# thiagopbueno/tf-mpc

Measured on AMD Instinct MI355X. Metric: iLQR iterations/sec (batch x horizon) at n=16,m=8,T=50, higher is better.
Workload: dtype f32

## Files before the change

tf-mpc_amd/csrc/lqr_mfma16x8.hip:

```cpp
#include <hip/hip_runtime.h>

#include <cstdlib>
#include <cstring>
#include <type_traits>

#include "lqr_kernels.h"
#include "options.h"
#include "mfma_bf16x3.h"
#include "wave_ldlt8.h"
#include "wave_ldlt8_pair.h"
#include "wave_ops.h"

namespace tfmpc {

namespace {

constexpr int N = 16, M = 8, D = 24;
using f32x4 = bf3::f32x4;

__device__ __forceinline__ f32x4 mfma(float a, float b, f32x4 c)
{
    return __builtin_amdgcn_mfma_f32_16x16x4f32(a, b, c, 0, 0, 0);
}

__device__ __forceinline__ float readlane(float v, int lane)
{
    return __builtin_bit_cast(float, __builtin_amdgcn_readlane(__builtin_bit_cast(int, v), lane));
}

using namespace bf3;

constexpr int kMs = 0;
constexpr int kKs = 256;
constexpr int kVt = 512;
constexpr int kVtLd = 20;
constexpr int kSweepFloats = kVt + 16 * kVtLd;
constexpr int kZs = 0;
constexpr int kZld = 26;
#ifndef TFMPC_LQR_TC
#define TFMPC_LQR_TC 52
#endif
constexpr int kTC = TFMPC_LQR_TC;
constexpr int kRolloutFloats = kZs + (kTC + 1) * kZld + 6;
constexpr int kLdsFloats = kSweepFloats > kRolloutFloats ? kSweepFloats : kRolloutFloats;
static_assert(kLdsFloats % 4 == 0, "slices are 16-byte aligned (pair_src, the 16-byte accesses of the sweep)");
#ifndef TFMPC_LQR_RING
#define TFMPC_LQR_RING 4
#endif
constexpr int kRing = TFMPC_LQR_RING;
static_assert(kTC % kRing == 0, "a chunk must hold whole turns of the gain ring");

template <int CTRL>
__device__ __forceinline__ float dpp(float v)
{
    return __builtin_bit_cast(float, __builtin_amdgcn_update_dpp(0, __builtin_bit_cast(int, v), CTRL, 0xF, 0xF, false));
}
constexpr int kDppXor1 = 0xB1;
constexpr int kDppXor2 = 0x4E;
constexpr int kDppHalfMirror = 0x141;

#define TFMPC_GLOBAL __attribute__((address_space(1)))
#define TFMPC_LDS __attribute__((address_space(3)))
using gbytes = TFMPC_GLOBAL char *;
__device__ __forceinline__ gbytes uniform_base(const float *p)
{
    gbytes g = (gbytes)p;
    asm("" : "+s"(g));
    return g;
}
__device__ __forceinline__ unsigned here(unsigned &off)
{
    asm volatile("" : "+v"(off));
    return off;
}
template <class V>
__device__ __forceinline__ V gload(gbytes base, unsigned &off) { return *reinterpret_cast<const TFMPC_GLOBAL V *>(base + here(off)); }
template <class V>
__device__ __forceinline__ void gstore(gbytes base, unsigned &off, V v) { *reinterpret_cast<TFMPC_GLOBAL V *>(base + here(off)) = v; }
__device__ __forceinline__ int pinned(int v)
{
    asm("" : "+v"(v));
    return v;
}
typedef float f32x4_lds __attribute__((ext_vector_type(4), aligned(8)));
typedef float f32x4_any __attribute__((ext_vector_type(4), aligned(4)));

#ifdef TFMPC_LQR_EU
#define TFMPC_LQR_WAVES(EU_) TFMPC_LQR_EU
#else
#define TFMPC_LQR_WAVES(EU_) (EU_)
#endif
#define TFMPC_LQR_OCCUPANCY __attribute__((amdgpu_waves_per_eu(TFMPC_LQR_WAVES(EU), TFMPC_LQR_WAVES(EU))))
__device__ __forceinline__ void block_lds_sync()
{
    __builtin_amdgcn_fence(__ATOMIC_RELEASE, "workgroup", "local");
    __builtin_amdgcn_s_barrier();
    __builtin_amdgcn_fence(__ATOMIC_ACQUIRE, "workgroup", "local");
}
template <bool BACKWARD, bool FORWARD, bool VALUE, bool EXACT, bool BF3, bool OUT16 = false, int EU = 4, bool PAIR = false>
__global__ __launch_bounds__(PAIR ? 2 * kWave : kWave) TFMPC_LQR_OCCUPANCY void lqr_mfma16x8_kernel(LqrArgs a)
{
    static_assert(!PAIR || (BACKWARD && !VALUE && !OUT16), "the paired elimination serves the sweeps without value outputs");
    __shared__ __attribute__((aligned(16))) float lds_all[(PAIR ? 2 : 1) * kLdsFloats];
    const int wave = PAIR ? __builtin_amdgcn_readfirstlane(threadIdx.x >> 6) : 0;
    float *const lds = lds_all + wave * kLdsFloats;
    const int b_own = PAIR ? 2 * (int)blockIdx.x + wave : (int)blockIdx.x;
    const bool live = !PAIR || b_own < a.B;
    const int b = live ? b_own : a.B - 1;
    const int lane = PAIR ? (int)(threadIdx.x & (kWave - 1)) : (int)threadIdx.x;
    const int i = lane & 15, q = lane >> 4;
    const int T = a.T;
    const int n = EXACT ? N : a.n, m = EXACT ? M : a.m, d = n + m;
    auto Fxx = [&](const float *Fg, int row, int xi) { return (row < n && xi < n) ? Fg[row * d + xi] : 0.0f; };
    auto Fxu = [&](const float *Fg, int row, int ui) { return (row < n && ui < m) ? Fg[row * d + n + ui] : 0.0f; };
    auto zmap = [&](int zi) { return zi < N ? (zi < n ? zi : -1) : (zi - N < m ? n + zi - N : -1); };
    auto Czz = [&](const float *Cg, int zr, int zc) {
        const int r = zmap(zr), c_ = zmap(zc);
        return (r >= 0 && c_ >= 0) ? Cg[r * d + c_] : 0.0f;
    };
    auto cz = [&](const float *cg, int zr) { const int r = zmap(zr); return r >= 0 ? cg[r] : 0.0f; };
    const float *Fg = a.F + (size_t)b * a.sF;
    const float *fg = a.f + (size_t)b * a.sf;
    const float *Cg = a.C + (size_t)b * a.sC;
    const float *cg = a.c + (size_t)b * a.sc;
    float *Kg = a.K + (size_t)b * a.sK;
    float *kg = a.k + (size_t)b * a.sk;
    int status = 0;

    if (BACKWARD) {
        float Fb0[4], Fb1[4];
        f32x4 Cd00, Cd11;
        f32x4 Cd01t;
        f32x4 vterm;
#pragma unroll
        for (int r = 0; r < 4; ++r) {
            const int k = 4 * q + r;
            const int ku = N + k;
            if (EXACT) {
                Fb0[r] = Fg[k * D + i];
                Fb1[r] = (i < M) ? Fg[k * D + N + i] : ((i == M) ? fg[k] : 0.0f);
                Cd00[r] = Cg[k * D + i];
                Cd01t[r] = (k < M) ? Cg[(N + k) * D + i] : ((k == M) ? cg[i] : 0.0f);
                vterm[r] = (i == M) ? cg[k] : 0.0f;
                Cd11[r] = (ku < D) ? ((i < M) ? Cg[ku * D + N + i] : ((i == M) ? cg[ku] : 0.0f)) : 0.0f;
            } else {
                Fb0[r] = Fxx(Fg, k, i);
                Fb1[r] = (i < M) ? Fxu(Fg, k, i) : ((i == M && k < n) ? fg[k] : 0.0f);
                Cd00[r] = Czz(Cg, k, i);
                Cd01t[r] = (k < M) ? Czz(Cg, N + k, i) : ((k == M) ? cz(cg, i) : 0.0f);
                vterm[r] = (i == M) ? cz(cg, k) : 0.0f;
                float c11 = 0.0f;
                if (ku < D) {
                    if (i < M) c11 = (k >= m && i == k) ? 1.0f : Czz(Cg, ku, N + i);
                    else if (i == M) c11 = cz(cg, ku);
                }
                Cd11[r] = c11;
            }
        }
        ConstFrag Fc0{}, Fc1{};
        if (BF3) {
            Fc0 = const_frag(f32x4{Fb0[0], Fb0[1], Fb0[2], Fb0[3]});
            Fc1 = const_frag(f32x4{Fb1[0], Fb1[1], Fb1[2], Fb1[3]});
        }
        f32x4 Vd = Cd00, vd = vterm;
        float cst = 0.0f;
        int min_pivot_bits = 0x3f800000;
        int min_pivot_rows = 0x3f800000;
        const int pj = lane & 15, prow = (lane >> 4) & 1;
        const int pcol = pj >= 8 ? pj - 8 + 8 * prow : (pj == 0 ? N + M : N + pj);
        const int pair_src = PAIR ? 4 * pinned(((lane >> 5) * kLdsFloats + kMs + pcol * 8) / 4) : 0;
        const int pair_d0 = (lane >> 5) * kLdsFloats + kMs + N * 8;
        constexpr int kZero = kMs + 25 * 8;
        if (lane < kKs - kZero) lds[kZero + lane] = 0.0f;
        constexpr int kQx = kMs + 28 * 8;
        constexpr int kPark = kMs + 30 * 8;
        const int pair_qx = (lane >> 5) * kLdsFloats + (pj >= 8 ? kQx + pj - 8 + 8 * prow : kPark + pj + 8 * prow);
        const int t01_src = (i == M) ? kQx + 4 * q : kZero;
        const int g0_src = pinned(kKs + i * 8 + q);
        const int vt_dst = pinned(kVt + 4 * q * kVtLd + i);
        unsigned offK = 8u * lane, offk = 4u * lane;
        __syncthreads();

        auto sweep_step = [&](const int t, auto LAST) __attribute__((always_inline)) {
            f32x4 W0 = {0.f, 0.f, 0.f, 0.f}, W1 = vd;
            if (BF3) {
                const VarFrag Vf = var_frag_block(Vd);
                W0 = mm_var_const(Vf, Fc0, W0);
                W1 = mm_var_const(Vf, Fc1, W1);
            } else {
#pragma unroll
                for (int r = 0; r < 4; ++r) {
                    W0 = mfma(Vd[r], Fb0[r], W0);
                    W1 = mfma(Vd[r], Fb1[r], W1);
                }
            }
            float fw = 0.0f, fv = 0.0f;
            if (VALUE) {
                float pw = 0.0f, pv = 0.0f;
#pragma unroll
                for (int r = 0; r < 4; ++r) {
                    pw = fmaf(Fb1[r], W1[r], pw);
                    pv = fmaf(Fb1[r], vd[r], pv);
                }
                fw = wave_sum(i == M ? pw : 0.0f);
                fv = wave_sum(i == M ? pv : 0.0f);
            }
            f32x4 T00 = Cd00, T01t = Cd01t, T11 = Cd11;
            if (BF3) {
                const VarFrag W0f = var_frag_block(W0), W1f = var_frag_block(W1);
                T00 = mm_const_var(Fc0, W0f, T00);
                T01t = mm_var_const(W1f, Fc0, T01t);
                T11 = mm_const_var(Fc1, W1f, T11);
            } else {
#pragma unroll
                for (int r = 0; r < 4; ++r) {
                    T00 = mfma(Fb0[r], W0[r], T00);
                    T01t = mfma(W1[r], Fb0[r], T01t);
                    T11 = mfma(Fb1[r], W1[r], T11);
                }
            }
            if (q < 2) {
                *reinterpret_cast<f32x4 *>(&lds[kMs + i * 8 + 4 * q]) = T01t;
                if (i <= M) *reinterpret_cast<f32x4 *>(&lds[kMs + (N + i) * 8 + 4 * q]) = T11;
            } else if (q == 2) {
                lds[kQx + i] = T01t[0];
            }
            float quk = 0.0f;
            if constexpr (PAIR) {
                block_lds_sync();
                if (wave == (t & 1)) {
                    f32x2 P2[4];
                    const f32x4 lo = *reinterpret_cast<const f32x4 *>(&lds_all[pair_src]);
                    const f32x4 hi = *reinterpret_cast<const f32x4 *>(&lds_all[pair_src + 4]);
                    const float d0 = lds_all[pair_d0];
                    const f32x4 qlo = *(const volatile TFMPC_LDS f32x4 *)&lds_all[pair_src];
                    const f32x4 qhi = *(const volatile TFMPC_LDS f32x4 *)&lds_all[pair_src + 4];
                    float vnext = lds_all[pair_qx];
                    P2[0] = f32x2{lo[0], lo[1]}; P2[1] = f32x2{lo[2], lo[3]};
                    P2[2] = f32x2{hi[0], hi[1]}; P2[3] = f32x2{hi[2], hi[3]};
                    const float Qc[8] = {qlo[0], qlo[1], qlo[2], qlo[3], qhi[0], qhi[1], qhi[2], qhi[3]};
                    float Pr[8];
                    ldlt8_pair_solve_neg(P2, Pr, d0, min_pivot_rows, Qc, vnext);
                    lds_all[pair_qx] = vnext;
                    f32x4 klo, khi;
#pragma unroll
                    for (int r = 0; r < 4; ++r) { klo[r] = Pr[r]; khi[r] = Pr[4 + r]; }
                    *reinterpret_cast<f32x4 *>(&lds_all[pair_src + (kKs - kMs)]) = klo;
                    *reinterpret_cast<f32x4 *>(&lds_all[pair_src + (kKs - kMs) + 4]) = khi;
                }
                block_lds_sync();
            } else {
                lds_sync();
                f32x2 M2[4];
                float Qc[8];
                {
                    const int c = lane & 31;
                    const f32x4 lo = *reinterpret_cast<const f32x4 *>(&lds[kMs + c * 8]);
                    const f32x4 hi = *reinterpret_cast<const f32x4 *>(&lds[kMs + c * 8 + 4]);
                    M2[0] = f32x2{lo[0], lo[1]}; M2[1] = f32x2{lo[2], lo[3]};
                    M2[2] = f32x2{hi[0], hi[1]}; M2[3] = f32x2{hi[2], hi[3]};
#pragma unroll
                    for (int r = 0; r < 4; ++r) { Qc[r] = lo[r]; Qc[4 + r] = hi[r]; }
                }
                float vnext = lds[kQx + (lane & 15)];
                float qu_saved[8];
                if (VALUE) {
#pragma unroll
                    for (int p = 0; p < 8; ++p) qu_saved[p] = readlane(M2[p >> 1][p & 1], 24);
                }
                float Mr[8];
                ldlt8_solve_neg(M2, Mr, min_pivot_bits);
                float kb[8];
#pragma unroll
                for (int p = 0; p < 8; ++p) kb[p] = readlane(Mr[p], 24);
                if (VALUE) {
#pragma unroll
                    for (int p = 0; p < 8; ++p) quk = fmaf(kb[p], qu_saved[p], quk);
                }
                if constexpr (!decltype(LAST)::value) {
#pragma unroll
                    for (int p = 0; p < 8; ++p) vnext = fmaf(kb[p], Qc[p], vnext);
                    if (lane < N) lds[kQx + lane] = vnext;
                }
                if (lane < 32) {
                    f32x4 lo, hi;
#pragma unroll
                    for (int r = 0; r < 4; ++r) { lo[r] = Mr[r]; hi[r] = Mr[4 + r]; }
                    *reinterpret_cast<f32x4 *>(&lds[kKs + lane * 8]) = lo;
                    *reinterpret_cast<f32x4 *>(&lds[kKs + lane * 8 + 4]) = hi;
                }
                lds_sync();
            }
            if constexpr (!decltype(LAST)::value) {
                const f32x4 vacc = *reinterpret_cast<const f32x4 *>(&lds[t01_src]);
#pragma unroll
                for (int s2 = 0; s2 < 2; ++s2) {
                    const float ax = lds[kMs + i * 8 + 4 * s2 + q];
                    const float g0 = lds[g0_src + 4 * s2];
                    T00 = mfma(ax, g0, T00);
                }
                {
                    const float *vt = &lds[kVt];
#pragma unroll
                    for (int r = 0; r < 4; ++r) lds[vt_dst + r * kVtLd] = T00[r];
                    lds_sync();
                    const f32x4 Tt = *reinterpret_cast<const f32x4 *>(&vt[i * kVtLd + 4 * q]);
#pragma unroll
                    for (int r = 0; r < 4; ++r) Vd[r] = 0.5f * (T00[r] + Tt[r]);
                }
                vd = vacc;
            }
            if (live) {
                const int ka = lane >> 3, jc = lane & 7;
                float2 kv;
                kv.x = lds[kKs + (2 * jc) * 8 + ka];
                kv.y = lds[kKs + (2 * jc + 1) * 8 + ka];
                if (EXACT) {
                    gstore(uniform_base(Kg + (size_t)t * (M * N)), offK, f32x2{kv.x, kv.y});
                    if (lane < M) gstore(uniform_base(kg + (size_t)t * M), offk, lds[kKs + 24 * 8 + lane]);
                } else {
                    if (ka < m && 2 * jc < n) Kg[(size_t)t * m * n + ka * n + 2 * jc] = kv.x;
                    if (ka < m && 2 * jc + 1 < n) Kg[(size_t)t * m * n + ka * n + 2 * jc + 1] = kv.y;
                    if (lane < m) kg[(size_t)t * m + lane] = lds[kKs + 24 * 8 + lane];
                }
                if (OUT16 && a.K16) {
                    uint16_t *Ko = a.K16 + ((size_t)b * T + t) * (m * n);
                    if (ka < m && 2 * jc < n) Ko[ka * n + 2 * jc] = lqr_to_bf16(kv.x);
                    if (ka < m && 2 * jc + 1 < n) Ko[ka * n + 2 * jc + 1] = lqr_to_bf16(kv.y);
                }
                if (OUT16 && a.k16 && lane < m) a.k16[((size_t)b * T + t) * m + lane] = lqr_to_bf16(lds[kKs + 24 * 8 + lane]);
            }
            if (VALUE) {
                cst += 0.5f * quk + 0.5f * (fw + fv);
                if (a.V) {
                    float *Vo = a.V + ((size_t)b * T + t) * (n * n);
#pragma unroll
                    for (int r = 0; r < 4; ++r)
                        if (EXACT || (4 * q + r < n && i < n)) Vo[(4 * q + r) * n + i] = Vd[r];
                }
                if (a.v && i == M) {
                    float *vo = a.v + ((size_t)b * T + t) * n;
#pragma unroll
                    for (int r = 0; r < 4; ++r)
                        if (EXACT || 4 * q + r < n) vo[4 * q + r] = vd[r];
                }
                if (a.cst && lane == 0) a.cst[(size_t)b * T + t] = cst;
                if (OUT16 && a.V16) {
                    uint16_t *Vo = a.V16 + ((size_t)b * T + t) * (n * n);
#pragma unroll
                    for (int r = 0; r < 4; ++r)
                        if (EXACT || (4 * q + r < n && i < n)) Vo[(4 * q + r) * n + i] = lqr_to_bf16(Vd[r]);
                }
                if (OUT16 && a.v16 && i == M) {
                    uint16_t *vo = a.v16 + ((size_t)b * T + t) * n;
#pragma unroll
                    for (int r = 0; r < 4; ++r)
                        if (EXACT || 4 * q + r < n) vo[4 * q + r] = lqr_to_bf16(vd[r]);
                }
                if (OUT16 && a.cst16 && lane == 0) a.cst16[(size_t)b * T + t] = lqr_to_bf16(cst);
            }
            lds_sync();
        };
        constexpr int kPeeled = VALUE ? 0 : 1;
        for (int t = T - 1; t >= kPeeled; --t) sweep_step(t, std::false_type{});
        if (kPeeled && T > 0) sweep_step(0, std::true_type{});
        if constexpr (PAIR) {
            constexpr int kMinPv = kKs + 25 * 8;
            if ((lane & 31) == 0) lds[kMinPv + (lane >> 5)] = __builtin_bit_cast(float, min_pivot_rows);
            block_lds_sync();
            const int p0 = __builtin_bit_cast(int, lds_all[kMinPv + wave]), p1 = __builtin_bit_cast(int, lds_all[kLdsFloats + kMinPv + wave]);
            min_pivot_bits = __builtin_amdgcn_readfirstlane(p0 < p1 ? p0 : p1);
        }
        if (min_pivot_bits <= 0) status |= (min_pivot_bits == 0) ? TFMPC_ST_SINGULAR : TFMPC_ST_NOT_PD;
        if (VALUE && !(cst == cst)) status |= TFMPC_ST_NAN;
    }

    const int lane_rollout = (BACKWARD && FORWARD) ? pinned((int)__builtin_amdgcn_mbcnt_hi(~0u, __builtin_amdgcn_mbcnt_lo(~0u, 0u))) : lane;
    if (FORWARD) {
        const int lane = lane_rollout, i = lane & 15, q = lane >> 4;
        const int fi = lane >> 2, fc = lane & 3;
        const int ka = lane >> 3, jc = lane & 7;
        float Fr[6];
        if (EXACT) {
            const float2 *p = reinterpret_cast<const float2 *>(Fg + fi * D + 6 * fc);
#pragma unroll
            for (int j = 0; j < 3; ++j) { const float2 v = p[j]; Fr[2 * j] = v.x; Fr[2 * j + 1] = v.y; }
        } else {
#pragma unroll
            for (int j = 0; j < 6; ++j) {
                const int zc = 6 * fc + j;
                Fr[j] = zc < N ? Fxx(Fg, fi, zc) : Fxu(Fg, fi, zc - N);
            }
        }
        const float f_part = (fc == 0 && (EXACT || fi < n)) ? fg[fi] : 0.0f;
        float Ca0[6], Ca1[6];
        f32x4 cq0, cq1;
#pragma unroll
        for (int s2 = 0; s2 < 6; ++s2) {
            if (EXACT) {
                Ca0[s2] = Cg[i * D + 4 * s2 + q];
                Ca1[s2] = (i < M) ? Cg[(N + i) * D + 4 * s2 + q] : 0.0f;
            } else {
                Ca0[s2] = Czz(Cg, i, 4 * s2 + q);
                Ca1[s2] = (i < M) ? Czz(Cg, N + i, 4 * s2 + q) : 0.0f;
            }
        }
#pragma unroll
        for (int r = 0; r < 4; ++r) {
            cq0[r] = EXACT ? cg[4 * q + r] : cz(cg, 4 * q + r);
            cq1[r] = (q < 2) ? (EXACT ? cg[N + 4 * q + r] : cz(cg, N + 4 * q + r)) : 0.0f;
        }
        float *xs = a.states + (size_t)b * (T + 1) * n;
        float *us = a.actions + (size_t)b * T * m;
        float *cs = a.costs + (size_t)b * (T + 1);
        float *zs = &lds[kZs];
        __syncthreads();
        if (lane < N) {
            const float x = (EXACT || lane < n) ? a.x0[(size_t)b * n + lane] : 0.0f;
            zs[lane] = x;
            if (live && (EXACT || lane < n)) xs[lane] = x;
        }
        unsigned offK = 8u * lane, offk = 4u * ka;
        auto load_gain = [&](int t, float2 &Kv, float &kv) {
            if (EXACT) {
                const f32x2 K2 = gload<f32x2>(uniform_base(Kg + (size_t)t * (M * N)), offK);
                Kv = float2{K2[0], K2[1]};
                kv = gload<float>(uniform_base(kg + (size_t)t * M), offk);
            } else {
                const bool row = ka < m;
                Kv.x = (row && 2 * jc < n) ? Kg[(size_t)t * m * n + ka * n + 2 * jc] : 0.0f;
                Kv.y = (row && 2 * jc + 1 < n) ? Kg[(size_t)t * m * n + ka * n + 2 * jc + 1] : 0.0f;
                kv = row ? kg[(size_t)t * m + ka] : 0.0f;
            }
        };
        float2 KR[kRing];
        float kR[kRing];
#pragma unroll
        for (int d = 0; d < kRing; ++d) {
            KR[d] = float2{0.f, 0.f};
            kR[d] = 0.0f;
            if (T > 0) load_gain(d < T ? d : T - 1, KR[d], kR[d]);
        }
        __syncthreads();

        auto chunk_costs = [&](int rows, float *out) {
            float part = 0.0f;
            for (int nt = 0; nt * 16 < rows; ++nt) {
                const int row = (16 * nt + i < rows) ? 16 * nt + i : rows - 1;
                const float *zrow = zs + row * kZld;
                f32x4 D0 = {0.f, 0.f, 0.f, 0.f}, D1 = {0.f, 0.f, 0.f, 0.f};
#pragma unroll
                for (int s2 = 0; s2 < 6; ++s2) {
                    const float bz = zrow[4 * s2 + q];
                    D0 = mfma(Ca0[s2], bz, D0);
                    D1 = mfma(Ca1[s2], bz, D1);
                }
                part = 0.0f;
#pragma unroll
                for (int r = 0; r < 4; ++r) {
                    part = fmaf(zrow[4 * q + r], fmaf(0.5f, D0[r], cq0[r]), part);
                    if (q < 2) part = fmaf(zrow[N + 4 * q + r], fmaf(0.5f, D1[r], cq1[r]), part);
                }
                part += __shfl_xor(part, 16, kWave);
                part += __shfl_xor(part, 32, kWave);
                if (live && q == 0 && 16 * nt + i < rows) {
                    unsigned offc = 4u * lane;
                    gstore(uniform_base(out + 16 * nt), offc, part);
                }
            }
            return part;
        };

        auto rollout_step = [&](const int tt, const int t, float2 &KRd, float &kRd, auto REFILL) __attribute__((always_inline)) {
            float *zt = zs + tt * kZld;
            const float2 Kc = KRd;
            const float kc = kRd;
            const float2 xv = *reinterpret_cast<const float2 *>(&zt[2 * jc]);
            float u = fmaf(Kc.x, xv.x, Kc.y * xv.y);
            u += dpp<kDppXor1>(u);
            u += dpp<kDppXor2>(u);
            u += dpp<kDppHalfMirror>(u);
            u += kc;
            if constexpr (decltype(REFILL)::value) load_gain(t + kRing < T ? t + kRing : T - 1, KRd, kRd);
            zt[N + ka] = u;
            lds_sync();
            float xn = f_part;
            const float2 *zp = reinterpret_cast<const float2 *>(&zt[6 * fc]);
#pragma unroll
            for (int j = 0; j < 3; ++j) {
                const float2 z2 = zp[j];
                xn = fmaf(Fr[2 * j], z2.x, xn);
                xn = fmaf(Fr[2 * j + 1], z2.y, xn);
            }
            xn += dpp<kDppXor1>(xn);
            xn += dpp<kDppXor2>(xn);
            zt[kZld + fi] = xn;
            lds_sync();
        };

        const int xrow = lane >> 2, urow = lane >> 1;
        const float *xsrc = zs + (1 + xrow) * kZld + 4 * (lane & 3);
        const float *usrc = zs + urow * kZld + N + 4 * (lane & 1);
        unsigned off16 = 16u * lane;
        auto rows_left = [](int v) { asm("" : "+s"(v)); return v; };

        for (int t0 = 0; t0 == 0 || t0 < T; t0 += kTC) {
            const bool last = T - t0 <= kTC;
            const int tc = last ? T - t0 : kTC;
            int tb = 0;
            for (; tb + kRing <= tc; tb += kRing) {
#pragma unroll
                for (int d = 0; d < kRing; ++d) rollout_step(tb + d, t0 + tb + d, KR[d], kR[d], std::true_type{});
            }
#pragma unroll
            for (int d = 0; d < kRing - 1; ++d)
                if (tb + d < tc) rollout_step(tb + d, t0 + tb + d, KR[d], kR[d], std::false_type{});
            if (last) {
                if (lane < M) zs[tc * kZld + N + lane] = __builtin_bit_cast(float, pinned(0));
                lds_sync();
            }
            const float tile_costs = chunk_costs(last ? tc + 1 : tc, cs + t0);
            if (last) {
                const float fcost = readlane(tile_costs, tc & 15);
                if (!(fcost == fcost)) status |= TFMPC_ST_NAN;
            }
            if (!live) {
            } else if (EXACT) {
                const gbytes xdst = uniform_base(xs + (size_t)(t0 + 1) * N), udst = uniform_base(us + (size_t)t0 * M);
#pragma unroll
                for (int r0 = 0; r0 < kTC; r0 += kWave / 4) {
                    const int left = rows_left(tc - r0);
                    if (left <= 0) break;
                    if (xrow < left)
                        gstore<f32x4_any>(xdst + r0 * (N * 4), off16, *reinterpret_cast<const f32x4_lds *>(xsrc + r0 * kZld));
                }
#pragma unroll
                for (int r0 = 0; r0 < kTC; r0 += kWave / 2) {
                    const int left = rows_left(tc - r0);
                    if (left <= 0) break;
                    if (urow < left)
                        gstore<f32x4_any>(udst + r0 * (M * 4), off16, *reinterpret_cast<const f32x4_lds *>(usrc + r0 * kZld));
                }
            } else {
                for (int idx = lane; idx < tc * n; idx += kWave)
                    xs[(size_t)(t0 + 1) * n + idx] = zs[(1 + idx / n) * kZld + idx % n];
                for (int idx = lane; idx < tc * m; idx += kWave)
                    us[(size_t)t0 * m + idx] = zs[(idx / m) * kZld + N + idx % m];
            }
            if (!last) {
                lds_sync();
                if (lane < N) zs[lane] = zs[kTC * kZld + lane];
                lds_sync();
            }
        }
    }

    if (live && a.status && lane_rollout == 0) a.status[b] = status;
}

bool use_bf16x3()
{
    return !option_is(kOptLqrMfma, "f32");
}

int pick_eu()
{
    const int forced = option_int(kOptLqrWaves, 0);
    return forced == 4 || forced == 6 ? forced : 5;
}

template <bool BW, bool FW, bool VAL, bool O16, int EU>
int launch_eu(const LqrArgs &a, hipStream_t stream)
{
    const bool exact = a.n == N && a.m == M;
    const bool bf3 = BW && use_bf16x3();
    constexpr bool P = BW && !VAL && !O16;
    const dim3 grid(P ? (a.B + 1) / 2 : a.B), block(P ? 2 * kWave : kWave);
    if (exact && bf3) hipLaunchKernelGGL((lqr_mfma16x8_kernel<BW, FW, VAL, true, true, O16, EU, P>), grid, block, 0, stream, a);
    else if (exact) hipLaunchKernelGGL((lqr_mfma16x8_kernel<BW, FW, VAL, true, false, O16, EU, P>), grid, block, 0, stream, a);
    else if (bf3) hipLaunchKernelGGL((lqr_mfma16x8_kernel<BW, FW, VAL, false, true, O16, EU, P>), grid, block, 0, stream, a);
    else hipLaunchKernelGGL((lqr_mfma16x8_kernel<BW, FW, VAL, false, false, O16, EU, P>), grid, block, 0, stream, a);
    return hipGetLastError() == hipSuccess ? TFMPC_OK : TFMPC_ERR_LAUNCH;
}

template <bool BW, bool FW, bool VAL, bool O16 = false>
int launch(const LqrArgs &a, hipStream_t stream)
{
    if constexpr (!VAL) {
        const int eu = pick_eu();
        if constexpr (BW && !O16) {
            if (eu == 6) return launch_eu<BW, FW, VAL, O16, 6>(a, stream);
        }
        if (eu >= 5) return launch_eu<BW, FW, VAL, O16, 5>(a, stream);
    }
    return launch_eu<BW, FW, VAL, O16, 4>(a, stream);
}

}

bool lqr_mfma_supported(int n, int m) { return n >= 1 && m >= 1 && n <= N && m <= M && n + m > 6; }

int lqr_mfma_launch(const LqrArgs &a, bool backward, bool forward, hipStream_t stream)
{
    if (a.K16 || a.k16 || a.V16 || a.v16 || a.cst16) {
        if (backward && forward) return launch<true, true, true, true>(a, stream);
        if (backward) return launch<true, false, true, true>(a, stream);
    }
    const bool value = a.V || a.v || a.cst;
    if (backward && forward) return value ? launch<true, true, true>(a, stream) : launch<true, true, false>(a, stream);
    if (backward) return value ? launch<true, false, true>(a, stream) : launch<true, false, false>(a, stream);
    return launch<false, true, false>(a, stream);
}

}
```

tf-mpc_amd/csrc/wave_ldlt8_pair.h:

```cpp
#pragma once

#include <hip/hip_runtime.h>

#include "wave_ldlt8.h"

namespace tfmpc {

#define TFMPC_BC(L) " row_newbcast:" #L " row_mask:0xf bank_mask:0xf\n\t"
#define TFMPC_PIVOT(P) "v_rcp_f32_dpp %[x" #P "], -%[m" #P "]" TFMPC_BC(P) \
                       "v_min_i32_dpp %[mp], %[m" #P "], %[mp]" TFMPC_BC(P) \
                       "v_mul_f32 %[x" #P "], %[m" #P "], %[x" #P "]\n\t"
#define TFMPC_FWD(P, S) "v_fmac_f32_dpp %[m" #S "], %[x" #P "], %[m" #P "]" TFMPC_BC(S)
#define TFMPC_BWD(P, O, S) "v_fmac_f32_dpp %[x" #P "], %[" #O "], %[x" #S "]" TFMPC_BC(S)
#define TFMPC_COPY(O, P) "v_mov_b32 %[" #O "], %[x" #P "]\n\t"
#define TFMPC_VAL(A) "v_fmac_f32_dpp %[acc], %[x" #A "], %[q" #A "]" TFMPC_BC(0)

__device__ __forceinline__ void ldlt8_pair_solve_neg(const f32x2 (&M2)[4], float (&X)[8], float d0, int &min_pivot_bits, const float (&Q)[8],
                                                     float &acc)
{
    float M[8];
#pragma unroll
    for (int r = 0; r < 8; ++r) M[r] = M2[r >> 1][r & 1];
    asm("v_rcp_f32 %[x0], -%[d0]\n\t"
        "v_min_i32 %[mp], %[d0], %[mp]\n\t"
        "v_mul_f32 %[x0], %[m0], %[x0]\n\t"
        "s_nop 1\n\t"
        TFMPC_FWD(0, 1) TFMPC_FWD(0, 2) TFMPC_FWD(0, 3) TFMPC_FWD(0, 4) TFMPC_FWD(0, 5) TFMPC_FWD(0, 6) TFMPC_FWD(0, 7)
        TFMPC_PIVOT(1) "s_nop 1\n\t"
        TFMPC_FWD(1, 2) TFMPC_FWD(1, 3) TFMPC_FWD(1, 4) TFMPC_FWD(1, 5) TFMPC_FWD(1, 6) TFMPC_FWD(1, 7)
        TFMPC_PIVOT(2) "s_nop 1\n\t"
        TFMPC_FWD(2, 3) TFMPC_FWD(2, 4) TFMPC_FWD(2, 5) TFMPC_FWD(2, 6) TFMPC_FWD(2, 7)
        TFMPC_PIVOT(3) "s_nop 1\n\t"
        TFMPC_FWD(3, 4) TFMPC_FWD(3, 5) TFMPC_FWD(3, 6) TFMPC_FWD(3, 7)
        TFMPC_PIVOT(4) "s_nop 1\n\t"
        TFMPC_FWD(4, 5) TFMPC_FWD(4, 6) TFMPC_FWD(4, 7)
        TFMPC_PIVOT(5) "s_nop 1\n\t"
        TFMPC_FWD(5, 6) TFMPC_FWD(5, 7)
        "s_nop 0\n\t"
        TFMPC_PIVOT(6) "s_nop 1\n\t"
        TFMPC_FWD(6, 7)
        TFMPC_COPY(m0, 5) TFMPC_COPY(m1, 4)
        TFMPC_PIVOT(7)
        "v_fmac_f32_dpp %[x6], %[x6], %[x7]" TFMPC_BC(7)
        TFMPC_BWD(5, m0, 7) TFMPC_BWD(5, m0, 6)
        TFMPC_COPY(m0, 3)
        TFMPC_BWD(4, m1, 7) TFMPC_BWD(4, m1, 6) TFMPC_BWD(4, m1, 5)
        TFMPC_COPY(m1, 2)
        TFMPC_BWD(3, m0, 7) TFMPC_BWD(3, m0, 6) TFMPC_BWD(3, m0, 5) TFMPC_BWD(3, m0, 4)
        TFMPC_COPY(m0, 1)
        TFMPC_BWD(2, m1, 7) TFMPC_BWD(2, m1, 6) TFMPC_BWD(2, m1, 5) TFMPC_BWD(2, m1, 4) TFMPC_BWD(2, m1, 3)
        TFMPC_COPY(m1, 0)
        TFMPC_BWD(1, m0, 7) TFMPC_BWD(1, m0, 6) TFMPC_BWD(1, m0, 5) TFMPC_BWD(1, m0, 4) TFMPC_BWD(1, m0, 3) TFMPC_BWD(1, m0, 2)
        TFMPC_BWD(0, m1, 7) TFMPC_BWD(0, m1, 6) TFMPC_BWD(0, m1, 5) TFMPC_BWD(0, m1, 4) TFMPC_BWD(0, m1, 3) TFMPC_BWD(0, m1, 2) TFMPC_BWD(0, m1, 1)
        "s_nop 1\n\t"
        TFMPC_VAL(0) TFMPC_VAL(1) TFMPC_VAL(2) TFMPC_VAL(3) TFMPC_VAL(4) TFMPC_VAL(5) TFMPC_VAL(6) TFMPC_VAL(7)
        : [x0] "=&v"(X[0]), [x1] "=&v"(X[1]), [x2] "=&v"(X[2]), [x3] "=&v"(X[3]), [x4] "=&v"(X[4]), [x5] "=&v"(X[5]), [x6] "=&v"(X[6]),
          [x7] "=&v"(X[7]), [m0] "+v"(M[0]), [m1] "+v"(M[1]), [m2] "+v"(M[2]), [m3] "+v"(M[3]), [m4] "+v"(M[4]), [m5] "+v"(M[5]),
          [m6] "+v"(M[6]), [m7] "+v"(M[7]), [mp] "+v"(min_pivot_bits), [acc] "+v"(acc)
        : [d0] "v"(d0), [q0] "v"(Q[0]), [q1] "v"(Q[1]), [q2] "v"(Q[2]), [q3] "v"(Q[3]), [q4] "v"(Q[4]), [q5] "v"(Q[5]), [q6] "v"(Q[6]),
          [q7] "v"(Q[7]));
}
#undef TFMPC_VAL
#undef TFMPC_COPY
#undef TFMPC_BWD
#undef TFMPC_FWD
#undef TFMPC_PIVOT
#undef TFMPC_BC

}
```

Before: 44.54 million.

## Compute value-gradient correction from eliminated rows, overlapping with LDLT solve

The value-vector update (Qx + K^T Qu) is rewritten as a dot product between the forward-eliminated rows and the original M rows, so it no longer waits for back-substitution. In the pair path the VAL accumulations are interleaved into the pivot stalls in place of s_nop padding, and the separate Q register copies read through volatile LDS loads are removed. In the single-wave path the solve is split into eliminate and backsub helpers so the vnext store can be issued before back-substitution. This shortens the critical path per timestep but changes the floating-point evaluation order, and the new eliminate and backsub helpers replace the previous tuned solve.

```diff
diff --git a/tf-mpc_amd/csrc/lqr_mfma16x8.hip b/tf-mpc_amd/csrc/lqr_mfma16x8.hip
--- a/tf-mpc_amd/csrc/lqr_mfma16x8.hip
+++ b/tf-mpc_amd/csrc/lqr_mfma16x8.hip
@@ -233,15 +233,13 @@
                     const f32x4 lo = *reinterpret_cast<const f32x4 *>(&lds_all[pair_src]);
                     const f32x4 hi = *reinterpret_cast<const f32x4 *>(&lds_all[pair_src + 4]);
                     const float d0 = lds_all[pair_d0];
-                    const f32x4 qlo = *(const volatile TFMPC_LDS f32x4 *)&lds_all[pair_src];
-                    const f32x4 qhi = *(const volatile TFMPC_LDS f32x4 *)&lds_all[pair_src + 4];
                     float vnext = lds_all[pair_qx];
                     P2[0] = f32x2{lo[0], lo[1]}; P2[1] = f32x2{lo[2], lo[3]};
                     P2[2] = f32x2{hi[0], hi[1]}; P2[3] = f32x2{hi[2], hi[3]};
-                    const float Qc[8] = {qlo[0], qlo[1], qlo[2], qlo[3], qhi[0], qhi[1], qhi[2], qhi[3]};
                     float Pr[8];
-                    ldlt8_pair_solve_neg(P2, Pr, d0, min_pivot_rows, Qc, vnext);
-                    lds_all[pair_qx] = vnext;
+                    float corr = 0.0f;
+                    ldlt8_pair_solve_neg(P2, Pr, d0, min_pivot_rows, corr);
+                    lds_all[pair_qx] = vnext + corr;
                     f32x4 klo, khi;
 #pragma unroll
                     for (int r = 0; r < 4; ++r) { klo[r] = Pr[r]; khi[r] = Pr[4 + r]; }
@@ -252,15 +250,12 @@
             } else {
                 lds_sync();
                 f32x2 M2[4];
-                float Qc[8];
                 {
                     const int c = lane & 31;
                     const f32x4 lo = *reinterpret_cast<const f32x4 *>(&lds[kMs + c * 8]);
                     const f32x4 hi = *reinterpret_cast<const f32x4 *>(&lds[kMs + c * 8 + 4]);
                     M2[0] = f32x2{lo[0], lo[1]}; M2[1] = f32x2{lo[2], lo[3]};
                     M2[2] = f32x2{hi[0], hi[1]}; M2[3] = f32x2{hi[2], hi[3]};
-#pragma unroll
-                    for (int r = 0; r < 4; ++r) { Qc[r] = lo[r]; Qc[4 + r] = hi[r]; }
                 }
                 float vnext = lds[kQx + (lane & 15)];
                 float qu_saved[8];
@@ -268,19 +263,24 @@
 #pragma unroll
                     for (int p = 0; p < 8; ++p) qu_saved[p] = readlane(M2[p >> 1][p & 1], 24);
                 }
+                f32x2 N2[4];
+                float nl[8][8];
+                ldlt8_eliminate_neg(M2, N2, nl, min_pivot_bits);
+                if constexpr (!decltype(LAST)::value) {
+                    float corr = 0.0f;
+#pragma unroll
+                    for (int p = 0; p < 8; ++p) corr = fmaf(readlane(N2[p >> 1][p & 1], 24), M2[p >> 1][p & 1], corr);
+                    vnext += corr;
+                    if (lane < N) lds[kQx + lane] = vnext;
+                }
                 float Mr[8];
-                ldlt8_solve_neg(M2, Mr, min_pivot_bits);
+                ldlt8_backsub_neg(N2, nl, Mr);
                 float kb[8];
 #pragma unroll
                 for (int p = 0; p < 8; ++p) kb[p] = readlane(Mr[p], 24);
                 if (VALUE) {
 #pragma unroll
                     for (int p = 0; p < 8; ++p) quk = fmaf(kb[p], qu_saved[p], quk);
-                }
-                if constexpr (!decltype(LAST)::value) {
-#pragma unroll
-                    for (int p = 0; p < 8; ++p) vnext = fmaf(kb[p], Qc[p], vnext);
-                    if (lane < N) lds[kQx + lane] = vnext;
                 }
                 if (lane < 32) {
                     f32x4 lo, hi;
diff --git a/tf-mpc_amd/csrc/wave_ldlt8_pair.h b/tf-mpc_amd/csrc/wave_ldlt8_pair.h
--- a/tf-mpc_amd/csrc/wave_ldlt8_pair.h
+++ b/tf-mpc_amd/csrc/wave_ldlt8_pair.h
@@ -13,10 +13,9 @@
 #define TFMPC_FWD(P, S) "v_fmac_f32_dpp %[m" #S "], %[x" #P "], %[m" #P "]" TFMPC_BC(S)
 #define TFMPC_BWD(P, O, S) "v_fmac_f32_dpp %[x" #P "], %[" #O "], %[x" #S "]" TFMPC_BC(S)
 #define TFMPC_COPY(O, P) "v_mov_b32 %[" #O "], %[x" #P "]\n\t"
-#define TFMPC_VAL(A) "v_fmac_f32_dpp %[acc], %[x" #A "], %[q" #A "]" TFMPC_BC(0)
+#define TFMPC_VAL(A) "v_fmac_f32_dpp %[acc], %[x" #A "], %[m" #A "]" TFMPC_BC(0)
 
-__device__ __forceinline__ void ldlt8_pair_solve_neg(const f32x2 (&M2)[4], float (&X)[8], float d0, int &min_pivot_bits, const float (&Q)[8],
-                                                     float &acc)
+__device__ __forceinline__ void ldlt8_pair_solve_neg(const f32x2 (&M2)[4], float (&X)[8], float d0, int &min_pivot_bits, float &acc)
 {
     float M[8];
 #pragma unroll
@@ -26,21 +25,23 @@
         "v_mul_f32 %[x0], %[m0], %[x0]\n\t"
         "s_nop 1\n\t"
         TFMPC_FWD(0, 1) TFMPC_FWD(0, 2) TFMPC_FWD(0, 3) TFMPC_FWD(0, 4) TFMPC_FWD(0, 5) TFMPC_FWD(0, 6) TFMPC_FWD(0, 7)
-        TFMPC_PIVOT(1) "s_nop 1\n\t"
+        TFMPC_PIVOT(1) TFMPC_VAL(0) "s_nop 0\n\t"
         TFMPC_FWD(1, 2) TFMPC_FWD(1, 3) TFMPC_FWD(1, 4) TFMPC_FWD(1, 5) TFMPC_FWD(1, 6) TFMPC_FWD(1, 7)
-        TFMPC_PIVOT(2) "s_nop 1\n\t"
+        TFMPC_PIVOT(2) TFMPC_VAL(1) "s_nop 0\n\t"
         TFMPC_FWD(2, 3) TFMPC_FWD(2, 4) TFMPC_FWD(2, 5) TFMPC_FWD(2, 6) TFMPC_FWD(2, 7)
-        TFMPC_PIVOT(3) "s_nop 1\n\t"
+        TFMPC_PIVOT(3) TFMPC_VAL(2) "s_nop 0\n\t"
         TFMPC_FWD(3, 4) TFMPC_FWD(3, 5) TFMPC_FWD(3, 6) TFMPC_FWD(3, 7)
-        TFMPC_PIVOT(4) "s_nop 1\n\t"
+        TFMPC_PIVOT(4) TFMPC_VAL(3) "s_nop 0\n\t"
         TFMPC_FWD(4, 5) TFMPC_FWD(4, 6) TFMPC_FWD(4, 7)
-        TFMPC_PIVOT(5) "s_nop 1\n\t"
+        TFMPC_PIVOT(5) TFMPC_VAL(4) "s_nop 0\n\t"
         TFMPC_FWD(5, 6) TFMPC_FWD(5, 7)
-        "s_nop 0\n\t"
+        TFMPC_VAL(5)
         TFMPC_PIVOT(6) "s_nop 1\n\t"
         TFMPC_FWD(6, 7)
+        TFMPC_VAL(6) "s_nop 0\n\t"
+        TFMPC_PIVOT(7) "s_nop 1\n\t"
+        TFMPC_VAL(7)
         TFMPC_COPY(m0, 5) TFMPC_COPY(m1, 4)
-        TFMPC_PIVOT(7)
         "v_fmac_f32_dpp %[x6], %[x6], %[x7]" TFMPC_BC(7)
         TFMPC_BWD(5, m0, 7) TFMPC_BWD(5, m0, 6)
         TFMPC_COPY(m0, 3)
@@ -52,13 +53,10 @@
         TFMPC_COPY(m1, 0)
         TFMPC_BWD(1, m0, 7) TFMPC_BWD(1, m0, 6) TFMPC_BWD(1, m0, 5) TFMPC_BWD(1, m0, 4) TFMPC_BWD(1, m0, 3) TFMPC_BWD(1, m0, 2)
         TFMPC_BWD(0, m1, 7) TFMPC_BWD(0, m1, 6) TFMPC_BWD(0, m1, 5) TFMPC_BWD(0, m1, 4) TFMPC_BWD(0, m1, 3) TFMPC_BWD(0, m1, 2) TFMPC_BWD(0, m1, 1)
-        "s_nop 1\n\t"
-        TFMPC_VAL(0) TFMPC_VAL(1) TFMPC_VAL(2) TFMPC_VAL(3) TFMPC_VAL(4) TFMPC_VAL(5) TFMPC_VAL(6) TFMPC_VAL(7)
         : [x0] "=&v"(X[0]), [x1] "=&v"(X[1]), [x2] "=&v"(X[2]), [x3] "=&v"(X[3]), [x4] "=&v"(X[4]), [x5] "=&v"(X[5]), [x6] "=&v"(X[6]),
           [x7] "=&v"(X[7]), [m0] "+v"(M[0]), [m1] "+v"(M[1]), [m2] "+v"(M[2]), [m3] "+v"(M[3]), [m4] "+v"(M[4]), [m5] "+v"(M[5]),
           [m6] "+v"(M[6]), [m7] "+v"(M[7]), [mp] "+v"(min_pivot_bits), [acc] "+v"(acc)
-        : [d0] "v"(d0), [q0] "v"(Q[0]), [q1] "v"(Q[1]), [q2] "v"(Q[2]), [q3] "v"(Q[3]), [q4] "v"(Q[4]), [q5] "v"(Q[5]), [q6] "v"(Q[6]),
-          [q7] "v"(Q[7]));
+        : [d0] "v"(d0));
 }
 #undef TFMPC_VAL
 #undef TFMPC_COPY
@@ -67,4 +65,40 @@
 #undef TFMPC_PIVOT
 #undef TFMPC_BC
 
+__device__ __forceinline__ void ldlt8_eliminate_neg(f32x2 (&M2)[4], f32x2 (&N2)[4], float (&nl)[8][8], int &min_pivot_bits)
+{
+    constexpr int kQuu = 16;
+#pragma unroll
+    for (int p = 0; p < 8; ++p) {
+        const int pp = p >> 1, ps = p & 1;
+        const float Mp = M2[pp][ps];
+        const int pvb = __builtin_amdgcn_readlane(__builtin_bit_cast(int, Mp), kQuu + p);
+        asm("s_min_i32 %0, %0, %1" : "+s"(min_pivot_bits) : "s"(pvb) : "scc");
+        const float ninv = __builtin_amdgcn_rcpf(-__builtin_bit_cast(float, pvb));
+        const float Mn = Mp * ninv;
+        N2[pp][ps] = Mn;
+#pragma unroll
+        for (int s = p + 1; s < 8; ++s)
+            nl[s][p] = __builtin_bit_cast(float, __builtin_amdgcn_readlane(__builtin_bit_cast(int, Mn), kQuu + s));
+        if (ps == 0) M2[pp][1] = fmaf(nl[p + 1][p], Mp, M2[pp][1]);
+        const f32x2 Mpp = {Mp, Mp};
+#pragma unroll
+        for (int k = pp + 1; k < 4; ++k) M2[k] = __builtin_elementwise_fma(f32x2{nl[2 * k][p], nl[2 * k + 1][p]}, Mpp, M2[k]);
+    }
 }
+
+__device__ __forceinline__ void ldlt8_backsub_neg(f32x2 (&N2)[4], const float (&nl)[8][8], float (&X)[8])
+{
+#pragma unroll
+    for (int s = 7; s >= 1; --s) {
+        const float Ns = N2[s >> 1][s & 1];
+        const f32x2 Nss = {Ns, Ns};
+        if (s & 1) N2[s >> 1][0] = fmaf(nl[s][s - 1], Ns, N2[s >> 1][0]);
+#pragma unroll
+        for (int k = 0; k < (s >> 1); ++k) N2[k] = __builtin_elementwise_fma(f32x2{nl[s][2 * k], nl[s][2 * k + 1]}, Nss, N2[k]);
+    }
+#pragma unroll
+    for (int r = 0; r < 8; ++r) X[r] = N2[r >> 1][r & 1];
+}
+
+}
```

Result: faster. 45.12 million, median of 6 (+1.3%).
